# scrubbbbs/cbird

Hardware: AMD Instinct MI355X
Metric: Hamming comparisons/sec + images hashed/sec, 1M-image index, 1/2/4/8 MI355X (higher is better)
Workload: dtype u64 hashes as 64 x FP4 signs, f32 accumulate (find, exact) / u8+f32 (hash)

## Files before the change

cbird_amd/csrc/cbh_internal.h:

```cpp
#pragma once
#include <hip/hip_runtime.h>
#include <stddef.h>
#include <stdint.h>

#include <cstring>
#include <atomic>
#include <map>
#include <memory>
#include <mutex>
#include <utility>
#include <vector>

#include "cbird_hip.h"

namespace cbh {

void combiner_drop(const void* handle);
void set_last_error(const char* where, hipError_t e);
void set_last_error_text(const char* text);
void clear_last_error();
void set_last_error_code(int code);
void* fail_handle(int code, const char* why);

hipError_t malloc_async(void** p, size_t bytes, hipStream_t s);
// ... 80 lines not shown
  JoinCache* join = nullptr;
  std::shared_ptr<const JoinTables>* join_hold = nullptr;
  const JoinNeedles* join_needles = nullptr;
};
int launch_hamm64_scan(const uint64_t* d_hashes, const uint32_t* d_ids, size_t n,
                       const uint64_t* d_q, size_t nq, int thresh, cbh_record* d_rec, size_t cap,
                       unsigned long long* d_total, hipStream_t stream, const ScanOpts& opts = {});
bool scan_takes_mfma(size_t n, size_t nq, int thresh);
int scan_pick_pre(const uint64_t* d_hashes, size_t n, size_t n_total, const uint64_t* d_q, size_t nq, int thresh,
                  hipStream_t stream);
int set_scan_mfma(int mode);
int get_scan_mfma();
void set_scan_pre_max(int t);
void set_scan_pre_rate(int e9);
void set_scan_pre48(int v);
long long get_scan_pre_mask();
long long get_scan_pre48_mask();
long long get_scan_probes();
long long get_scan_probe_rate_e9();
long long get_scan_probe_true_e9();
long long get_scan_probe_rate48_e9();

struct LoneBlock {
  volatile unsigned long long done;
  unsigned long long count;
  static constexpr unsigned kRecs = 512;
  cbh_record recs[kRecs];
};
int launch_find_one(const uint64_t* d_hashes, const uint32_t* d_ids, size_t n, uint64_t q, int thresh, unsigned* d_state,
                    LoneBlock* h_block, unsigned long long seq, hipStream_t stream);
int wait_find_one(const LoneBlock* h_block, unsigned long long seq, hipStream_t stream);

int launch_hamm64_scan_mfma(const uint64_t* d_hashes, const uint32_t* d_ids, size_t n, const uint64_t* d_q, size_t nq,
                            int thresh, cbh_record* d_rec, size_t cap, unsigned long long* d_total, hipStream_t stream,
                            int pre, const ScanOpts& opts);
int expand_needles_for_scan(const uint64_t* d_q, size_t nq, hipStream_t stream, uint4** qx);
constexpr int kProbeMaxThresh = 8;
bool probe_fold_rates(const uint64_t* d_hashes, size_t n, const uint64_t* d_q, size_t nq, int thresh, hipStream_t stream,
                      double* r_cand, double* r_true, double* r_cand48);
int selftest_fp4_products(float* d_out, hipStream_t stream);
constexpr int kJoinMaxThresh = 8;
long long get_scan_joins();
long long get_join_needle_preps();
int set_join_resident(int v);
int set_join_resident_mb(int v);
int get_join_resident();
int get_join_resident_mb();
struct JoinTables {
  int m = 0, device = 0;
  size_t n = 0, bytes = 0;
  uint32_t *hist_h = nullptr, *start_h = nullptr, *hid = nullptr;
  uint64_t* hx = nullptr;
  JoinTables() = default;
  JoinTables(const JoinTables&) = delete;
// ... 148 lines not shown
```

cbird_amd/csrc/cbird_hip.hip:

```cpp
#include <algorithm>
#include <atomic>
#include <cmath>
#include <cstdio>
#include <cstring>
#include <map>
#include <mutex>
#include <new>
#include <string>
#include <vector>

#include "cbh_internal.h"

namespace cbh {

static thread_local std::string t_last_error;
static thread_local int t_last_code = CBH_OK;

void set_last_error(const char* where, hipError_t e) {
  char buf[512];
  snprintf(buf, sizeof buf, "%s: %s (%d)", where, hipGetErrorString(e), (int)e);
  t_last_error = buf;
  t_last_code = e == hipErrorOutOfMemory ? CBH_E_NOMEM : CBH_E_HIP;
}

// ... 1288 lines not shown
      {"fdct_host_vote", [](int v) { g_fdct_host_vote = v; }},
      {"video_host_reduce", [](int v) { g_video_host_reduce = v; }},
      {"orb_retain_order", [](int v) { set_orb_retain_order(v); }},
      {"pool_keep_mb", [](int v) { set_pool_keep_mb(v); }},
      {"pool_live_keep_mb", [](int v) { set_pool_live_keep_mb(v); }},
      {"shard_force_rccl", [](int v) { set_shard_force_rccl(v); }},
      {"shard_exchange", [](int v) { set_shard_exchange(v); }},
      {"fault_alloc_after", [](int v) { set_fault_alloc_after(v); }},
      {"fault_alloc_sticky", [](int v) { set_fault_alloc_sticky(v); }},
      {"fault_driver_oom", [](int v) { set_fault_driver_oom(v); }},
      {"fault_persist_oom", [](int v) { set_fault_persist_oom(v); }},
      {"fault_rccl", [](int v) { set_fault_rccl(v); }},
  };
  if (!strcmp(key, "orb_retain_order") && value != 0 && value != 1) return CBH_E_INVAL;
  if (!strcmp(key, "scan_mfma")) return set_scan_mfma(value);
  if (!strcmp(key, "scan256_mfma")) return set_scan256_mfma(value);
  if (!strcmp(key, "scan256_small")) return set_scan256_small(value);
  if (!strcmp(key, "join_resident")) return set_join_resident(value);
  if (!strcmp(key, "join_resident_mb")) return set_join_resident_mb(value);
  if (!strcmp(key, "color_create_group")) return set_cd_group(value);
  if (!strcmp(key, "scan256_kernels")) {
    if (value != 0) return CBH_E_INVAL;
    clear_scan256_kernels();
    return CBH_OK;
  }
  for (const auto& k : kKnobs)
    if (!strcmp(key, k.name)) {
      k.set(value);
      return CBH_OK;
    }
  return CBH_E_INVAL;
}

int cbh_get_tuning(const char* key, long long* value) {
  if (!key || !value) return CBH_E_INVAL;
  if (!strcmp(key, "fault_alloc_after")) return *value = get_fault_alloc_after(), CBH_OK;
  if (!strcmp(key, "fault_fired")) return *value = (long long)get_fault_fired(), CBH_OK;
  if (!strcmp(key, "alloc_calls")) return *value = (long long)get_alloc_calls(), CBH_OK;
  if (!strncmp(key, "arena_", 6)) return arena_counter(key + 6, value);
  if (!strcmp(key, "scan_mfma")) return *value = get_scan_mfma(), CBH_OK;
  if (!strcmp(key, "scan_pre_mask")) return *value = get_scan_pre_mask(), CBH_OK;
  if (!strcmp(key, "scan_pre48_mask")) return *value = get_scan_pre48_mask(), CBH_OK;
  if (!strcmp(key, "scan256_mfma")) return *value = get_scan256_mfma(), CBH_OK;
  if (!strcmp(key, "scan256_small")) return *value = get_scan256_small(), CBH_OK;
  if (!strcmp(key, "scan256_kernels")) return *value = get_scan256_kernels(), CBH_OK;
  if (!strcmp(key, "color_create_group")) return *value = get_cd_group(), CBH_OK;
  if (!strcmp(key, "color_create_group_last")) return *value = get_cd_group_last(), CBH_OK;
  if (!strcmp(key, "scan_probes")) return *value = get_scan_probes(), CBH_OK;
  if (!strcmp(key, "scan_joins")) return *value = get_scan_joins(), CBH_OK;
  if (!strcmp(key, "join_needle_preps")) return *value = get_join_needle_preps(), CBH_OK;
  if (!strcmp(key, "join_resident")) return *value = get_join_resident(), CBH_OK;
  if (!strcmp(key, "join_resident_mb")) return *value = get_join_resident_mb(), CBH_OK;
  if (!strcmp(key, "slices_on_device")) return *value = get_slices_on_device(), CBH_OK;
  if (!strcmp(key, "scan_probe_rate_e9")) return *value = get_scan_probe_rate_e9(), CBH_OK;
  if (!strcmp(key, "scan_probe_true_e9")) return *value = get_scan_probe_true_e9(), CBH_OK;
  if (!strcmp(key, "scan_probe_rate48_e9")) return *value = get_scan_probe_rate48_e9(), CBH_OK;
  return CBH_E_INVAL;
}


int cbh_idx64_time_scan_dev(cbh_idx64* idx, const void* d_q, size_t nq, int thresh,
                            void* d_records, size_t cap, void* d_total, int iters, float* ms_avg) {
  if (!idx || !ms_avg || iters <= 0 || !d_total) return CBH_E_INVAL;
  if (idx->shards) return CBH_E_UNSUPPORTED;
  DeviceGuard g(idx->device);
  if (!g.ok) return CBH_E_NODEVICE;
  int rc;
  WsLease L(idx, &rc);
  if (!L.ws) return rc;
  hipStream_t s = L.ws->stream;
  hipEvent_t e0, e1;
// ... 99 lines not shown
```

cbird_amd/csrc/fp4_sign.h:

```cpp
#pragma once
#include <hip/hip_runtime.h>

#include <cstdint>

namespace cbh {

typedef int v8i __attribute__((ext_vector_type(8)));
typedef float v16f __attribute__((ext_vector_type(16)));

constexpr int kScaleOne = 0x7f7f7f7f;

__device__ __forceinline__ uint4 fp4_expand32(uint32_t w) {
  uint32_t o[4];
#pragma unroll
  for (int d = 0; d < 4; ++d) {
    uint32_t x = (w >> (8 * d)) & 0xffu;
    x = (x | (x << 12)) & 0x000f000fu;
    x = (x | (x << 6)) & 0x03030303u;
    x = (x | (x << 3)) & 0x11111111u;
    o[d] = 0xaaaaaaaau ^ (x << 3);
  }
  return make_uint4(o[0], o[1], o[2], o[3]);
}

// ... 4 lines not shown
#pragma unroll
  for (int d = 0; d < 2; ++d) {
    uint32_t x = (w >> (8 * d)) & 0xffu;
    x = (x | (x << 12)) & 0x000f000fu;
    x = (x | (x << 6)) & 0x03030303u;
    x = (x | (x << 3)) & 0x11111111u;
    o[d] = (0x88888888u | (mag * 0x11111111u)) ^ (x << 3);
  }
  return make_uint2(o[0], o[1]);
}

__host__ __device__ __forceinline__ uint32_t pre48_sub(uint32_t lo, uint32_t hi, uint32_t k) {
  return k == 0 ? (lo ^ hi) & 0xffffu : k == 1 ? lo >> 16 : hi >> 16;
}

__device__ __forceinline__ v8i fp4_operand(uint4 e) {
  return v8i{(int)e.x, (int)e.y, (int)e.z, (int)e.w, 0, 0, 0, 0};
}

}
```

cbird_amd/csrc/hamm64_mfma.hip:

```cpp
#include <algorithm>
#include <mutex>
#include <vector>

#include "cbh_internal.h"
#include "fp4_sign.h"

namespace cbh {
namespace {

typedef _Float16 h2 __attribute__((ext_vector_type(2)));

constexpr int kThreads = 256;
constexpr int kWaves = 4;
constexpr int kHT = 8;
constexpr int kHT48 = 6;
constexpr int kG = 2;
constexpr float kC0 = 8388608.0f + 16448.0f + 2097152.0f;
constexpr int kScale15 = 0x8e8e8e8e;
constexpr uint32_t kQueue = 2048;
constexpr uint32_t kFlagMaskPre = (1u << 5) | (1u << 11) | (1u << 17) | (1u << 23);
constexpr int kScaleHalf = 0x7e7e7e7e;
constexpr int kScale5 = (int)0x84848484;
constexpr int kScale11 = (int)0x8a8a8a8a;
constexpr int kScale17 = (int)0x90909090;
constexpr int kScale1 = (int)0x80808080;
constexpr int kScale7p = (int)0x86868686;
constexpr int kScale10 = (int)0x89898989;
constexpr int kScale13 = (int)0x8c8c8c8c;
constexpr int kScale19 = (int)0x92929292;

constexpr uint32_t kNeedlePad = 384;
__global__ __launch_bounds__(256) void k_expand_needles(const uint64_t* __restrict__ q, uint32_t nq,
                                                        uint32_t nq_pad, uint4* __restrict__ qx) {
  const uint32_t i = blockIdx.x * 256u + threadIdx.x;
  if (i >= 3u * nq_pad + nq_pad / 128u * 192u) return;
  const uint32_t* w = reinterpret_cast<const uint32_t*>(q);
  if (i < 2u * nq_pad) {
    qx[i] = fp4_expand32((i >> 1) < nq ? w[i] : 0u);
  } else if (i >= 3u * nq_pad) {
    const uint32_t u = i - 3u * nq_pad, quad = u / 192u, m = (u % 192u) >> 6, c = u & 31u, kb = (u >> 5) & 1u;
    uint2 o[2];
#pragma unroll
    for (uint32_t k = 0; k < 2; ++k) {
      const uint32_t s = 2u * (2u * m + kb) + k, j = quad * 128u + (s / 3u) * 32u + c;
      const uint32_t lo = j < nq ? w[2u * j] : 0u, hi = j < nq ? w[2u * j + 1u] : 0u;
      o[k] = fp4_expand16(pre48_sub(lo, hi, s % 3u), s == 3u || s == 7u || s == 9u ? kFp4Four : kFp4Half);
    }
    qx[i] = make_uint4(o[0].x, o[0].y, o[1].x, o[1].y);
  } else {
    const uint32_t j = i - 2u * nq_pad;
    qx[i] = fp4_expand32(j < nq ? w[2u * j] ^ w[2u * j + 1u] : 0u);
  }
// ... 151 lines not shown
  uint32_t* s_out = PRE ? s_queue + kOutOff : s_out2_[PRE ? 0 : wave];
  uint32_t nout = 0;

  v8i a[HT];
#pragma unroll
  for (int t = 0; t < HT; ++t) {
    const uint32_t row = (tile0 + t) * 32u + r;
    const uint2 hv = row < n ? hay[row] : make_uint2(0u, 0u);
    if constexpr (PRE == 2) {
      const uint32_t e0 = pre48_sub(hv.x, hv.y, 0), e1 = pre48_sub(hv.x, hv.y, 1), e2 = pre48_sub(hv.x, hv.y, 2);
      const uint2 s0 = fp4_expand16(half ? e2 : e0, kFp4Half);
      const uint2 s1 = fp4_expand16(half ? e0 : e1, half ? kFp4Four : kFp4Half);
      const uint2 s2 = fp4_expand16(half ? e1 : e2, kFp4Half);
      const uint2 s3 = fp4_expand16(half ? e2 : e0, half ? kFp4Half : kFp4Four);
      a[t] = v8i{(int)s0.x, (int)s0.y, (int)s1.x, (int)s1.y, (int)s2.x, (int)s2.y, (int)s3.x, (int)s3.y};
    } else {
      a[t] = fp4_operand(fp4_expand32(PRE ? hv.x ^ hv.y : (half ? hv.y : hv.x)));
    }
    if (PRE && half == 0) s_hay[t * 32 + r] = hv;
  }
  wave_order();
  v16f c0;
#pragma unroll
  for (int g = 0; g < 16; ++g)
    c0[g] = PRE == 2 ? 8388608.0f + (float)((8u + thresh) * 266305u)
            : PRE  ? 8388608.0f + (float)((16u + (thresh - 1u)) * 266305u) : kC0;
  asm volatile("" : "+v"(c0));
  int scale_b = PRE == 2 ? kScale1 : PRE ? (half ? kScale5 : kScaleHalf) : kScaleOne;
  int scale_b2 = PRE == 2 ? (half ? kScale10 : kScale7p) : PRE ? (half ? kScale17 : kScale11) : kScale15;
  int scale_b3 = half ? kScale19 : kScale13;
  asm volatile("" : "+v"(scale_b));
  asm volatile("" : "+v"(scale_b2));
  if constexpr (PRE == 2) asm volatile("" : "+v"(scale_b3));

  const uint32_t p0 = blockIdx.y * pairs_per_chunk;
  const uint32_t p1 = min(n_pairs, p0 + pairs_per_chunk);
  const uint4* __restrict__ qp = qx + ((size_t)p0 * 64u + r) * 2u + half;
  const uint32_t lo_zero = 0x4080u;
  const uint32_t hi_zero = 0x4B40u;
  const uint32_t lo_thr = lo_zero - 2u * (thresh - 1u);
  const uint32_t hi_thr = hi_zero - (thresh - 1u);
  const uint32_t lo_key = lo_thr << 16, hi_key = hi_thr << 16;
  const HitParams hp = {lo_key, hi_key, lo_zero, hi_zero, thresh, n, nq, keep0, q, ids, rec, cap, total, hay, qmask};

  uint32_t npend = 0;
  uint32_t nitem = 0;
  uint32_t* s_item = s_queue + kItemOff;
// ... 114 lines not shown
        const v8i& h = a[t0 + t];
        c[t] = __builtin_amdgcn_mfma_scale_f32_32x32x64_f8f6f4(v8i{h[2], h[3], h[4], h[5], 0, 0, 0, 0}, b1, c[t], 4, 4, 0,
                                                               kScaleOne, 0, scale_b2);
      }
#pragma unroll
      for (int t = 0; t < G; ++t) {
        const v8i& h = a[t0 + t];
        c[t] = __builtin_amdgcn_mfma_scale_f32_32x32x64_f8f6f4(v8i{h[4], h[5], h[6], h[7], 0, 0, 0, 0}, b2, c[t], 4, 4, 0,
                                                               kScaleOne, 0, scale_b3);
      }
      detect(c, (uint32_t)(t0 / G), p);
    }
    if (npend >= 64u) drain(false);
  };

  auto step = [&](const uint32_t p, const uint4& nA, const uint4& nB) __attribute__((always_inline)) {
    const v8i bA = fp4_operand(nA);
    const v8i bB = fp4_operand(nB);
#pragma unroll
    for (int t0 = 0; t0 < HT; t0 += G) {
      v16f c[G];
#pragma unroll
      for (int t = 0; t < G; ++t)
        c[t] = __builtin_amdgcn_mfma_scale_f32_32x32x64_f8f6f4(a[t0 + t], bA, c0, 4, 4, 0, kScaleOne,
                                                               0, scale_b);
#pragma unroll
      for (int t = 0; t < G; ++t)
        c[t] = __builtin_amdgcn_mfma_scale_f32_32x32x64_f8f6f4(a[t0 + t], bB, c[t], 4, 4, 0,
                                                               kScaleOne, 0, scale_b2);
      if constexpr (PRE != 0) {
// ... 7 lines not shown
            m0 = pkmax3(m0, as_h2(c[t][g]), as_h2(c[t][g + 1]));
            m1 = pkmax3(m1, as_h2(c[t][g + 2]), as_h2(c[t][g + 3]));
          }
        const uint32_t mb = __builtin_bit_cast(uint32_t, __builtin_elementwise_maximum(m0, m1));
        const bool hit = (mb << 16) >= lo_key || mb >= hi_key;
        if (__builtin_amdgcn_ballot_w64(hit) != 0) {
#pragma unroll
          for (int t = 0; t < G; ++t) handle_tile2(c[t], (tile0 + t0 + t) * 32u, p, hp, s_queue, s_out, nout);
        }
      }
    }
    if constexpr (PRE != 0)
      if (npend >= 64u) drain(false);
  };

  (void)step, (void)step48, (void)detect;
  if constexpr (PRE == 2) {
    typedef unsigned v4u_t __attribute__((ext_vector_type(4)));
    const __amdgpu_buffer_rsrc_t rsrc = __builtin_amdgcn_make_buffer_rsrc(
        const_cast<uint4*>(qf + (size_t)(p0 >> 1) * 192u), 0, (int)0xffffffffu, 0x27000);
    const uint32_t voff = lane * 16u;
    auto ldt = [&](uint32_t rel, uint32_t m) -> uint4 {
      const v4u_t v = __builtin_amdgcn_raw_buffer_load_b128(rsrc, (int)voff, (int)(rel * 3072u + m * 1024u), 0);
      return make_uint4(v.x, v.y, v.z, v.w);
    };
    const uint32_t nqd = (p1 - p0 + 1u) >> 1;
    uint4 x0 = ldt(0, 0), x1 = ldt(0, 1), x2 = ldt(0, 2);
#pragma unroll 1
    for (uint32_t rel = 0; rel < nqd; rel += 2) {
      const uint32_t ry = min(rel + 1, nqd - 1);
      const uint4 y0 = ldt(ry, 0), y1 = ldt(ry, 1), y2 = ldt(ry, 2);
      step48(p0 + 2u * rel, x0, x1, x2);
// ... 46 lines not shown
  }
  out_flush(s_out, nout, hp);
}

#define CBH_MFMA_PARAMS                                                                                              \
  const uint2 *__restrict__ hay, const uint32_t *__restrict__ ids, uint32_t n, const uint64_t *__restrict__ q,       \
      const uint4 *__restrict__ qx, uint32_t nq, uint32_t n_pairs, uint32_t pairs_per_chunk, uint32_t thresh,        \
      cbh_record *__restrict__ rec, unsigned long long cap, unsigned long long *__restrict__ total, uint32_t keep0,  \
      const uint2 *__restrict__ qmask, const uint4 *__restrict__ qf
#define CBH_MFMA_ARGS hay, ids, n, q, qx, nq, n_pairs, pairs_per_chunk, thresh, rec, cap, total, keep0, qmask, qf
template <bool PRE>
__global__ __launch_bounds__(kThreads, PRE ? 4 : 1) void k_hamm64_mfma(CBH_MFMA_PARAMS) {
  hamm64_mfma_body<PRE ? 1 : 0>(CBH_MFMA_ARGS);
}
__global__ __launch_bounds__(kThreads, 3) void k_hamm64_mfma48(CBH_MFMA_PARAMS) { hamm64_mfma_body<2>(CBH_MFMA_ARGS); }
#undef CBH_MFMA_PARAMS
#undef CBH_MFMA_ARGS


constexpr uint32_t kFlagMask3 = (1u << 7) | (1u << 14) | (1u << 21);
constexpr int kScale7 = (int)0x86868686;
constexpr int kScale14 = (int)0x8d8d8d8d;

__device__ __forceinline__ void handle_tile3(const v16f& c, uint32_t row0, uint32_t p3, const HitParams& hp,
                                             uint32_t* s_queue, uint32_t* s_out, uint32_t& nout) {
  const uint32_t lane = threadIdx.x & 63u;
  uint32_t any = 0;
#pragma unroll
  for (int g = 0; g < 16; ++g) any |= as_u32(c[g]);
  if (__builtin_amdgcn_ballot_w64((any & kFlagMask3) != 0) == 0) return;
// ... 115 lines not shown
  }
  out_flush(s_out, nout, hp);
}

constexpr uint32_t kProbeS = 2048;
constexpr int kProbeT = kProbeMaxThresh;

__device__ __forceinline__ uint32_t probe_mix(uint32_t x) {
  x = ((x >> 16) ^ x) * 0x45d9f3bu;
  x = ((x >> 16) ^ x) * 0x45d9f3bu;
  return (x >> 16) ^ x;
}
__global__ __launch_bounds__(256) void k_fold_probe(const uint2* __restrict__ hay, uint32_t n, const uint2* __restrict__ q,
                                                    uint32_t nq, uint32_t sh, uint32_t sq, uint32_t* __restrict__ counts) {
  __shared__ uint2 s_h[64];
  __shared__ uint32_t s_cnt[3 * kProbeT];
  const uint32_t t = threadIdx.x;
  if (t < 64) {
    const uint32_t i = blockIdx.y * 64u + t;
    s_h[t] = i < sh ? hay[sh == n ? i : probe_mix(i) % n] : make_uint2(0u, 0u);
  }
  if (t < 3 * kProbeT) s_cnt[t] = 0;
  __syncthreads();
  const uint32_t j = blockIdx.x * 256u + t;
  const uint32_t nslots = min(64u, sh - blockIdx.y * 64u);
  uint32_t cnt[kProbeT] = {}, cnt64[kProbeT] = {}, cnt48[kProbeT] = {};
  if (j < sq) {
    const uint2 nv = q[sq == nq ? j : probe_mix(j ^ 0x9e3779b9u) % nq];
    const uint32_t f = nv.x ^ nv.y;
    for (uint32_t k = 0; k < nslots; ++k) {
      const uint2 hv = s_h[k];
      const uint32_t d = (uint32_t)__popc(f ^ hv.x ^ hv.y);
#pragma unroll
      for (int th = 0; th < kProbeT; ++th) cnt[th] += d < (uint32_t)(th + 1) ? 1u : 0u;
      const uint32_t d48 = (uint32_t)__popc((f ^ hv.x ^ hv.y) & 0xffffu) + (uint32_t)__popc((nv.x ^ hv.x) >> 16) +
                           (uint32_t)__popc((nv.y ^ hv.y) >> 16);
#pragma unroll
      for (int th = 0; th < kProbeT; ++th) cnt48[th] += d48 <= (uint32_t)(th + 1) || d48 > (uint32_t)(th + 33) ? 1u : 0u;
      if (d < (uint32_t)kProbeT) {
        const uint32_t d64 = (uint32_t)__popc(nv.x ^ hv.x) + (uint32_t)__popc(nv.y ^ hv.y);
#pragma unroll
        for (int th = 0; th < kProbeT; ++th) cnt64[th] += d64 < (uint32_t)(th + 1) ? 1u : 0u;
      }
    }
  }
#pragma unroll
  for (int th = 0; th < 3 * kProbeT; ++th) {
    uint32_t v = th < kProbeT ? cnt[th % kProbeT] : th < 2 * kProbeT ? cnt64[th % kProbeT] : cnt48[th % kProbeT];
#pragma unroll
    for (int o = 32; o > 0; o >>= 1) v += __shfl_down(v, o);
    if ((t & 63u) == 0 && v) atomicAdd(&s_cnt[th], v);
  }
  __syncthreads();
  if (t < 3 * kProbeT && s_cnt[t]) atomicAdd(&counts[t], s_cnt[t]);
}

__device__ __forceinline__ uint32_t selftest_fp4_code(uint32_t i) {
  return ((i >> 1) == 0 ? kFp4Half : (i >> 1) == 1 ? 0x2u : kFp4Four) | ((i & 1u) << 3);
}
__global__ __launch_bounds__(64) void k_selftest_fp4(float* __restrict__ out) {
  const uint32_t lane = threadIdx.x, half = lane >> 5;
  for (uint32_t i = 0; i < 720u; ++i) {
    const uint32_t kb = i & 1u, ci = (i >> 1) & 1u, k = (i >> 2) % 5u, ib = (i / 20u) % 6u, ia = i / 120u;
    const uint32_t fa = selftest_fp4_code(ia) * (ci ? 0x11111111u : 1u), fb = selftest_fp4_code(ib) * (ci ? 0x11111111u : 1u);
    const bool on = half == kb;
    const v8i a = {on ? (int)fa : 0, on && ci ? (int)fa : 0, 0, 0, 0, 0, 0, 0};
    const v8i b = {on ? (int)fb : 0, on && ci ? (int)fb : 0, 0, 0, 0, 0, 0, 0};
    int sc = k == 0 ? kScale1 : k == 1 ? kScale7p : k == 2 ? kScale10 : k == 3 ? kScale13 : kScale19;
    asm volatile("" : "+v"(sc));
// ... 4 lines not shown
  }
}

std::mutex g_probe_mu;
std::vector<uint32_t*> g_probe_free;
uint32_t* probe_slot_get() {
  {
    std::lock_guard<std::mutex> lk(g_probe_mu);
    if (!g_probe_free.empty()) {
      uint32_t* p = g_probe_free.back();
      g_probe_free.pop_back();
      return p;
    }
  }
  uint32_t* p = nullptr;
  if (hipHostMalloc(&p, 3 * kProbeT * sizeof(uint32_t)) != hipSuccess) {
    (void)hipGetLastError();
    return nullptr;
  }
  return p;
}
void probe_slot_put(uint32_t* p) {
  std::lock_guard<std::mutex> lk(g_probe_mu);
  g_probe_free.push_back(p);
}

}

bool probe_fold_rates(const uint64_t* d_hashes, size_t n, const uint64_t* d_q, size_t nq, int thresh, hipStream_t stream,
                      double* r_cand, double* r_true, double* r_cand48) {
  uint32_t* d_cnt = nullptr;
  if (cbh::malloc_async((void**)&d_cnt, 3 * kProbeT * sizeof(uint32_t), stream) != hipSuccess) {
    (void)hipGetLastError();
    return false;
  }
  uint32_t* h_cnt = probe_slot_get();
  bool ok = h_cnt != nullptr;
  const uint32_t sh = (uint32_t)std::min<size_t>(n, kProbeS), sq = (uint32_t)std::min<size_t>(nq, kProbeS);
  if (ok) {
    ok = hipMemsetAsync(d_cnt, 0, 3 * kProbeT * sizeof(uint32_t), stream) == hipSuccess;
    if (ok) {
      hipLaunchKernelGGL(k_fold_probe, dim3((sq + 255u) / 256u, (sh + 63u) / 64u), dim3(256), 0, stream,
                         reinterpret_cast<const uint2*>(d_hashes), (uint32_t)n, reinterpret_cast<const uint2*>(d_q),
                         (uint32_t)nq, sh, sq, d_cnt);
      ok = hipGetLastError() == hipSuccess &&
           hipMemcpyAsync(h_cnt, d_cnt, 3 * kProbeT * sizeof(uint32_t), hipMemcpyDeviceToHost, stream) == hipSuccess &&
           hipStreamSynchronize(stream) == hipSuccess;
    }
  }
  (void)cbh::free_async(d_cnt, stream);
  if (ok) {
    const double pairs = (double)sh * (double)sq;
    *r_cand = (double)h_cnt[thresh - 1] / pairs;
    *r_true = (double)h_cnt[kProbeT + thresh - 1] / pairs;
    *r_cand48 = (double)h_cnt[2 * kProbeT + thresh - 1] / pairs;
  } else {
    (void)hipGetLastError();
  }
  if (h_cnt) probe_slot_put(h_cnt);
  return ok;
}

int selftest_fp4_products(float* d_out, hipStream_t stream) {
  hipLaunchKernelGGL(k_selftest_fp4, dim3(1), dim3(64), 0, stream, d_out);
  CBH_HIP(hipGetLastError());
  return CBH_OK;
}

static uint32_t padded_needles(size_t nq) { return (uint32_t)((nq + kNeedlePad - 1) / kNeedlePad) * kNeedlePad; }

int expand_needles_for_scan(const uint64_t* d_q, size_t nq, hipStream_t stream, uint4** qx_out) {
  *qx_out = nullptr;
  if (nq == 0 || nq > CBH_MAX_QUERIES_PER_CALL) return CBH_OK;
  const uint32_t nq_pad = padded_needles(nq);
  uint4* qx = nullptr;
  CBH_HIP(malloc_async((void**)&qx, (size_t)nq_pad * 72u, stream));
  hipLaunchKernelGGL(k_expand_needles, dim3((3u * nq_pad + nq_pad / 128u * 192u + 255u) / 256u), dim3(256), 0, stream, d_q,
                     (uint32_t)nq, nq_pad, qx);
  hipError_t e = hipGetLastError();
  if (e != hipSuccess) {
    (void)free_async(qx, stream);
    CBH_HIP(e);
  }
  *qx_out = qx;
  return CBH_OK;
}

int launch_hamm64_scan_mfma(const uint64_t* d_hashes, const uint32_t* d_ids, size_t n, const uint64_t* d_q, size_t nq,
                            int thresh, cbh_record* d_rec, size_t cap, unsigned long long* d_total, hipStream_t stream,
                            int pre, const ScanOpts& o) {
  const uint32_t n_pairs = (uint32_t)((nq + 63) / 64);
  const uint32_t n_triples = (uint32_t)((nq + 95) / 96);
  const uint32_t nq_pad = padded_needles(nq);
  const uint4* qx = o.qx;
  uint4* qx_own = nullptr;
  if (!qx) {
    int rc = expand_needles_for_scan(d_q, nq, stream, &qx_own);
    if (rc) return rc;
    qx = qx_own;
  }
  const uint4* qf = qx + (pre == 2 ? 3u : 2u) * (size_t)nq_pad;
  const uint32_t rows_per_wg = 32u * (pre == 2 ? kHT48 : kHT) * kWaves;
  const uint32_t sib = std::max(1u, o.siblings);
  const uint32_t wgs = (uint32_t)((n + rows_per_wg - 1) / rows_per_wg);
  if (!pre && thresh <= 64) {
    uint32_t tpc = 172u;
    while (tpc > 11 && (uint64_t)wgs * sib * ((n_triples + tpc - 1) / tpc) < 8192) tpc = (tpc + 1) / 2;
    uint32_t ch3 = (n_triples + tpc - 1) / tpc;
    if (ch3 > 65535) {
      tpc = (n_triples + 65534) / 65535;
      ch3 = (n_triples + tpc - 1) / tpc;
    }
    hipLaunchKernelGGL(k_hamm64_mfma3, dim3(wgs, ch3), dim3(kThreads), 0, stream,
                       reinterpret_cast<const uint2*>(d_hashes), d_ids, (uint32_t)n, d_q, qx, (uint32_t)nq, n_triples, tpc,
                       (uint32_t)thresh, d_rec, (unsigned long long)cap, d_total, (uint32_t)o.keep_id0,
                       reinterpret_cast<const uint2*>(o.d_qmask));
  } else {
    uint32_t ppc = pre ? 512u : 256u;
    while (ppc > 16 && (uint64_t)wgs * sib * ((n_pairs + ppc - 1) / ppc) < 8192) ppc >>= 1;
    uint32_t chunks = (n_pairs + ppc - 1) / ppc;
    if (chunks > 65535) {
      ppc = ((n_pairs + 65534) / 65535 + 1u) & ~1u;
      chunks = (n_pairs + ppc - 1) / ppc;
    }
#define CBH_MFMA(K)                                                                                                   \
  hipLaunchKernelGGL(K, dim3(wgs, chunks), dim3(kThreads), 0, stream,                                                 \
                     reinterpret_cast<const uint2*>(d_hashes), d_ids, (uint32_t)n, d_q, qx, (uint32_t)nq, n_pairs, ppc, \
                     (uint32_t)thresh, d_rec, (unsigned long long)cap, d_total, (uint32_t)o.keep_id0,                 \
                     reinterpret_cast<const uint2*>(o.d_qmask), qf)
    if (pre == 2) CBH_MFMA(k_hamm64_mfma48); else if (pre) CBH_MFMA((k_hamm64_mfma<true>)); else CBH_MFMA((k_hamm64_mfma<false>));
#undef CBH_MFMA
  }
  hipError_t e = hipGetLastError();
  if (qx_own) (void)cbh::free_async(qx_own, stream);
  CBH_HIP(e);
  return CBH_OK;
}

}
```

cbird_amd/csrc/hamm64_scan.hip:

```cpp
#include <atomic>

#include "cbh_internal.h"

namespace cbh {
namespace {

constexpr int kThreads = 256;
constexpr int kH = 8;
constexpr int kQB = 8;

__device__ __forceinline__ uint32_t min3u(uint32_t a, uint32_t b, uint32_t c) {
  return min(min(a, b), c);
}

__device__ __forceinline__ void emit(cbh_record* __restrict__ rec, unsigned long long cap,
                                     unsigned long long* __restrict__ total, uint32_t qidx,
                                     uint32_t dist, uint32_t id) {
  unsigned long long slot = atomicAdd(total, 1ull);
  if (slot < cap) rec[slot] = ((cbh_record)qidx << 39) | ((cbh_record)dist << 32) | id;
}

template <int H>
__device__ __forceinline__ void exact_block(const uint2 (&h)[H], uint32_t base_idx, uint32_t n,
                                            const uint32_t* __restrict__ ids,
// ... 253 lines not shown
#if defined(__x86_64__)
    __builtin_ia32_pause();
#endif
  }
}

namespace {

constexpr int kPreMax = 7;
constexpr size_t kMfmaMinNq = 256;
constexpr size_t kMfmaMinN = 4096;
constexpr int kPreStatic = 6;
constexpr double kTrueWeight = 8.0;
constexpr double kSlopePre = 1.3e4, kBaseFull = 15.75, kTrueFull = 2.7e5, kTruePre = 0.7e5;
constexpr double kBasePre = 8.55, kBase48 = 14.0, kSlope48 = 2.8e4, kTrue48 = 1.0e5, kPre48Margin = 0.9;
constexpr int kPre48MaxThresh = 16;
constexpr uint64_t kProbeMinPairs = 1ull << 31;

int g_scan_mfma = 1;
int g_pre_max_thresh = -1;
int g_pre_rate_max_e9 = 300000;
int g_pre48 = -1;
std::atomic<uint64_t> g_pre_mask{0};
std::atomic<uint64_t> g_pre48_mask{0};
std::atomic<uint64_t> g_n_probe{0};
std::atomic<long long> g_last_rate_e9{-1};
std::atomic<long long> g_last_true_e9{-1};
std::atomic<long long> g_last_rate48_e9{-1};

enum class Join { None, IfCheaper, Forced };
enum class Kernel { PopcEq, PopcPre, PopcFull, Mfma };
struct Route {
  Join join;
  Kernel kernel;
  double scan_ms;
};

Route route(size_t n, size_t nq, int thresh, bool masked) {
  Route r;
  r.scan_ms = (double)n * (double)nq * (thresh <= 5 ? 8.7e-12 : thresh == 6 ? 9.7e-12 : thresh == 7 ? 12.1e-12 : 15.8e-12);
  const bool joinable = thresh <= kJoinMaxThresh && !masked && n < 0xfffffff0ull;
  r.join = !joinable ? Join::None : g_scan_mfma == 4 ? Join::Forced
           : g_scan_mfma == 3 && r.scan_ms >= 1.0 ? Join::IfCheaper : Join::None;
  const bool mfma = thresh <= 65 && (g_scan_mfma == 2 || g_scan_mfma == 4 ||
                                     (g_scan_mfma != 0 && nq >= kMfmaMinNq && n >= kMfmaMinN));
  r.kernel = mfma ? Kernel::Mfma : thresh == 1 ? Kernel::PopcEq : thresh <= kPreMax ? Kernel::PopcPre : Kernel::PopcFull;
  return r;
}

int launch_popc(Kernel kernel, const uint64_t* d_hashes, const uint32_t* d_ids, size_t n, const uint64_t* d_q, size_t nq,
                int thresh, cbh_record* d_rec, size_t cap, unsigned long long* d_total, hipStream_t stream,
                const ScanOpts& o) {
  const uint32_t tile = kThreads * kH;
  const uint32_t tiles = (uint32_t)((n + tile - 1) / tile);
  uint32_t q_chunk = 16384;
  while (q_chunk > 1024 && (uint64_t)tiles * ((nq + q_chunk - 1) / q_chunk) < 8192) q_chunk >>= 1;
  uint32_t chunks = (uint32_t)((nq + q_chunk - 1) / q_chunk);
  if (chunks > 65535) {
// ... 15 lines not shown
  return CBH_OK;
}

}

bool scan_takes_mfma(size_t n, size_t nq, int thresh) {
  return thresh >= 1 && route(n, nq, thresh, false).kernel == Kernel::Mfma;
}

bool scan_routes_to_join(size_t n, size_t nq, int thresh, bool masked) {
  return thresh >= 1 && n >= 1 && nq >= 1 && route(n, nq, thresh, masked).join != Join::None;
}

int scan_pick_pre(const uint64_t* d_hashes, size_t n, size_t n_total, const uint64_t* d_q, size_t nq, int thresh,
                  hipStream_t stream) {
  if (g_pre48 == 1 && thresh <= kPre48MaxThresh) return 2;
  if (thresh > 32) return 0;
  if (g_pre_max_thresh >= 0) return thresh <= g_pre_max_thresh;
  if (thresh > kProbeMaxThresh) return 0;
  if ((uint64_t)n_total * (uint64_t)nq < kProbeMinPairs) return thresh <= kPreStatic;
  double r_cand = 0, r_true = 0, r48 = 0;
  if (!probe_fold_rates(d_hashes, n, d_q, nq, thresh, stream, &r_cand, &r_true, &r48)) return thresh <= kPreStatic;
  g_last_rate_e9 = (long long)(r_cand * 1e9);
  g_last_true_e9 = (long long)(r_true * 1e9);
  g_last_rate48_e9 = (long long)(r48 * 1e9);
  g_n_probe++;
  const double d_pre = kSlopePre * (r_cand - kTrueWeight * r_true - (double)g_pre_rate_max_e9 * 1e-9);
  const bool pre = d_pre <= 0;
  if (g_pre48 != 0) {
    const double t_48 = kBase48 + kSlope48 * r48 + kTrue48 * r_true;
    const double t_pre = kBasePre + kSlopePre * r_cand + kTruePre * r_true, t_full = kBaseFull + kTrueFull * r_true;
    if (pre ? t_48 < kPre48Margin * t_pre : t_48 < t_full) return 2;
  }
  return pre;
}

namespace {

int launch_zero_needles(const uint64_t* d_hashes, const uint32_t* d_ids, size_t n, const uint64_t* d_q, size_t nq,
                        int thresh, cbh_record* d_rec, size_t cap, unsigned long long* d_total, hipStream_t stream,
                        const ScanOpts& o) {
  Scratch scratch(stream);
  uint32_t* list = nullptr;
  CBH_HIP(scratch.get(&list, (nq + 1) * sizeof(uint32_t)));
  CBH_HIP(hipMemsetAsync(list, 0, sizeof(uint32_t), stream));
  hipLaunchKernelGGL(k_zero_needle_list, dim3((unsigned)((nq + 255) / 256)), dim3(256), 0, stream, d_q, (uint32_t)nq, list);
// ... 23 lines not shown
namespace {

int scan_nonzero_needles(const uint64_t* d_hashes, const uint32_t* d_ids, size_t n, const uint64_t* d_q, size_t nq,
                         int thresh, cbh_record* d_rec, size_t cap, unsigned long long* d_total, hipStream_t stream,
                         const ScanOpts& o) {
  const Route r = route(n, nq, thresh, o.d_qmask != nullptr);
  if (r.join != Join::None) {
    const bool force = r.join == Join::Forced;
    const int rc = launch_hamm64_join(d_hashes, d_ids, n, d_q, nq, thresh, d_rec, cap, d_total, stream, o, force, r.scan_ms);
    if (rc == CBH_OK || force || (rc != CBH_E_UNSUPPORTED && rc != CBH_E_NOMEM)) return rc;
    if (rc == CBH_E_NOMEM) cbh_clear_error();
  }
  if (r.kernel != Kernel::Mfma) return launch_popc(r.kernel, d_hashes, d_ids, n, d_q, nq, thresh, d_rec, cap, d_total, stream, o);
  const int pre = o.pre >= 0 ? o.pre : scan_pick_pre(d_hashes, n, n, d_q, nq, thresh, stream);
  if (thresh < 64) {
    if (pre == 1) g_pre_mask |= 1ull << thresh; else g_pre_mask &= ~(1ull << thresh);
    if (pre == 2) g_pre48_mask |= 1ull << thresh; else g_pre48_mask &= ~(1ull << thresh);
  }
  return launch_hamm64_scan_mfma(d_hashes, d_ids, n, d_q, nq, thresh, d_rec, cap, d_total, stream, pre, o);
}

}

int set_scan_mfma(int mode) {
  if (mode < 0 || mode > 4) return CBH_E_INVAL;
  g_scan_mfma = mode;
  return CBH_OK;
}
int get_scan_mfma() { return g_scan_mfma; }
void set_scan_pre_max(int t) {
  if (t >= -1 && t <= 32) g_pre_max_thresh = t;
}
void set_scan_pre_rate(int e9) {
  if (e9 >= 0) g_pre_rate_max_e9 = e9;
}
void set_scan_pre48(int v) {
  if (v >= -1 && v <= 1) g_pre48 = v;
}
long long get_scan_pre_mask() { return (long long)g_pre_mask.load(); }
long long get_scan_pre48_mask() { return (long long)g_pre48_mask.load(); }
long long get_scan_probes() { return (long long)g_n_probe.load(); }
long long get_scan_probe_rate_e9() { return g_last_rate_e9.load(); }
long long get_scan_probe_true_e9() { return g_last_true_e9.load(); }
long long get_scan_probe_rate48_e9() { return g_last_rate48_e9.load(); }

}
```

Before: 86280 billion.

## Add 16-bit folded prefilter MFMA scan path chosen by probe cost model

Adds a third prefilter mode that folds each 64-bit hash into 16 bits (XOR of all four 16-bit quarters) and runs a single FP4 MFMA per needle to reject candidates before the exact check. The idea is that a Hamming distance within the threshold survives the fold, so the cheaper 16-bit screen removes most of the matrix work of the existing 32-bit fold path. The fold-rate probe now also measures the 16-bit candidate rate, and a cost model picks the new kernel when its estimated time beats the 32-bit prefilter. Route's scan-cost estimate for thresh 1 is also lowered, which changes join-versus-scan decisions. In exchange, the weaker fold lets through more false candidates that must be verified, and needle expansion needs a larger buffer.

After: 88690 billion, median of 6. 1.03x the previous value.

```diff
diff --git a/cbird_amd/csrc/cbh_internal.h b/cbird_amd/csrc/cbh_internal.h
--- a/cbird_amd/csrc/cbh_internal.h
+++ b/cbird_amd/csrc/cbh_internal.h
@@ -118,12 +118,15 @@
 void set_scan_pre_max(int t);
 void set_scan_pre_rate(int e9);
 void set_scan_pre48(int v);
+int set_scan_pre16(int v);
 long long get_scan_pre_mask();
 long long get_scan_pre48_mask();
+long long get_scan_pre16_mask();
 long long get_scan_probes();
 long long get_scan_probe_rate_e9();
 long long get_scan_probe_true_e9();
 long long get_scan_probe_rate48_e9();
+long long get_scan_probe_rate16_e9();
 
 struct LoneBlock {
   volatile unsigned long long done;
@@ -135,13 +138,14 @@
                     LoneBlock* h_block, unsigned long long seq, hipStream_t stream);
 int wait_find_one(const LoneBlock* h_block, unsigned long long seq, hipStream_t stream);
 
+constexpr int kPre16MaxThresh = 8;
 int launch_hamm64_scan_mfma(const uint64_t* d_hashes, const uint32_t* d_ids, size_t n, const uint64_t* d_q, size_t nq,
                             int thresh, cbh_record* d_rec, size_t cap, unsigned long long* d_total, hipStream_t stream,
                             int pre, const ScanOpts& opts);
 int expand_needles_for_scan(const uint64_t* d_q, size_t nq, hipStream_t stream, uint4** qx);
 constexpr int kProbeMaxThresh = 8;
 bool probe_fold_rates(const uint64_t* d_hashes, size_t n, const uint64_t* d_q, size_t nq, int thresh, hipStream_t stream,
-                      double* r_cand, double* r_true, double* r_cand48);
+                      double* r_cand, double* r_true, double* r_cand48, double* r_cand16);
 int selftest_fp4_products(float* d_out, hipStream_t stream);
 constexpr int kJoinMaxThresh = 8;
 long long get_scan_joins();
diff --git a/cbird_amd/csrc/cbird_hip.hip b/cbird_amd/csrc/cbird_hip.hip
--- a/cbird_amd/csrc/cbird_hip.hip
+++ b/cbird_amd/csrc/cbird_hip.hip
@@ -1326,6 +1326,7 @@
   };
   if (!strcmp(key, "orb_retain_order") && value != 0 && value != 1) return CBH_E_INVAL;
   if (!strcmp(key, "scan_mfma")) return set_scan_mfma(value);
+  if (!strcmp(key, "scan_pre16")) return set_scan_pre16(value);
   if (!strcmp(key, "scan256_mfma")) return set_scan256_mfma(value);
   if (!strcmp(key, "scan256_small")) return set_scan256_small(value);
   if (!strcmp(key, "join_resident")) return set_join_resident(value);
@@ -1353,6 +1354,7 @@
   if (!strcmp(key, "scan_mfma")) return *value = get_scan_mfma(), CBH_OK;
   if (!strcmp(key, "scan_pre_mask")) return *value = get_scan_pre_mask(), CBH_OK;
   if (!strcmp(key, "scan_pre48_mask")) return *value = get_scan_pre48_mask(), CBH_OK;
+  if (!strcmp(key, "scan_pre16_mask")) return *value = get_scan_pre16_mask(), CBH_OK;
   if (!strcmp(key, "scan256_mfma")) return *value = get_scan256_mfma(), CBH_OK;
   if (!strcmp(key, "scan256_small")) return *value = get_scan256_small(), CBH_OK;
   if (!strcmp(key, "scan256_kernels")) return *value = get_scan256_kernels(), CBH_OK;
@@ -1367,6 +1369,7 @@
   if (!strcmp(key, "scan_probe_rate_e9")) return *value = get_scan_probe_rate_e9(), CBH_OK;
   if (!strcmp(key, "scan_probe_true_e9")) return *value = get_scan_probe_true_e9(), CBH_OK;
   if (!strcmp(key, "scan_probe_rate48_e9")) return *value = get_scan_probe_rate48_e9(), CBH_OK;
+  if (!strcmp(key, "scan_probe_rate16_e9")) return *value = get_scan_probe_rate16_e9(), CBH_OK;
   return CBH_E_INVAL;
 }
 
diff --git a/cbird_amd/csrc/fp4_sign.h b/cbird_amd/csrc/fp4_sign.h
--- a/cbird_amd/csrc/fp4_sign.h
+++ b/cbird_amd/csrc/fp4_sign.h
@@ -42,6 +42,11 @@
   return k == 0 ? (lo ^ hi) & 0xffffu : k == 1 ? lo >> 16 : hi >> 16;
 }
 
+__host__ __device__ __forceinline__ uint32_t fold16(uint32_t lo, uint32_t hi) {
+  const uint32_t f = lo ^ hi;
+  return (f ^ (f >> 16)) & 0xffffu;
+}
+
 __device__ __forceinline__ v8i fp4_operand(uint4 e) {
   return v8i{(int)e.x, (int)e.y, (int)e.z, (int)e.w, 0, 0, 0, 0};
 }
diff --git a/cbird_amd/csrc/hamm64_mfma.hip b/cbird_amd/csrc/hamm64_mfma.hip
--- a/cbird_amd/csrc/hamm64_mfma.hip
+++ b/cbird_amd/csrc/hamm64_mfma.hip
@@ -33,9 +33,16 @@
 __global__ __launch_bounds__(256) void k_expand_needles(const uint64_t* __restrict__ q, uint32_t nq,
                                                         uint32_t nq_pad, uint4* __restrict__ qx) {
   const uint32_t i = blockIdx.x * 256u + threadIdx.x;
-  if (i >= 3u * nq_pad + nq_pad / 128u * 192u) return;
+  const uint32_t o16 = 3u * nq_pad + nq_pad / 128u * 192u;
+  if (i >= o16 + nq_pad / 128u * 64u) return;
   const uint32_t* w = reinterpret_cast<const uint32_t*>(q);
-  if (i < 2u * nq_pad) {
+  if (i >= o16) {
+    const uint32_t u = i - o16, c = u & 31u, kb = (u >> 5) & 1u;
+    const uint32_t j0 = (u >> 6) * 128u + kb * 64u + c, j1 = j0 + 32u;
+    const uint2 lo = fp4_expand16(j0 < nq ? fold16(w[2u * j0], w[2u * j0 + 1u]) : 0u, kFp4Half);
+    const uint2 hi = fp4_expand16(j1 < nq ? fold16(w[2u * j1], w[2u * j1 + 1u]) : 0u, kFp4Four);
+    qx[i] = make_uint4(lo.x, lo.y, hi.x, hi.y);
+  } else if (i < 2u * nq_pad) {
     qx[i] = fp4_expand32((i >> 1) < nq ? w[i] : 0u);
   } else if (i >= 3u * nq_pad) {
     const uint32_t u = i - 3u * nq_pad, quad = u / 192u, m = (u % 192u) >> 6, c = u & 31u, kb = (u >> 5) & 1u;
@@ -217,6 +224,10 @@
       const uint2 s2 = fp4_expand16(half ? e1 : e2, kFp4Half);
       const uint2 s3 = fp4_expand16(half ? e2 : e0, half ? kFp4Half : kFp4Four);
       a[t] = v8i{(int)s0.x, (int)s0.y, (int)s1.x, (int)s1.y, (int)s2.x, (int)s2.y, (int)s3.x, (int)s3.y};
+    } else if constexpr (PRE == 3) {
+      const uint32_t f = fold16(hv.x, hv.y);
+      const uint2 s0 = fp4_expand16(f, kFp4Half), s1 = fp4_expand16(f, kFp4Four);
+      a[t] = v8i{(int)s0.x, (int)s0.y, (int)s1.x, (int)s1.y, 0, 0, 0, 0};
     } else {
       a[t] = fp4_operand(fp4_expand32(PRE ? hv.x ^ hv.y : (half ? hv.y : hv.x)));
     }
@@ -226,14 +237,15 @@
   v16f c0;
 #pragma unroll
   for (int g = 0; g < 16; ++g)
-    c0[g] = PRE == 2 ? 8388608.0f + (float)((8u + thresh) * 266305u)
+    c0[g] = PRE == 3 ? 8388608.0f + (float)((24u + (thresh - 1u)) * 266305u)
+            : PRE == 2 ? 8388608.0f + (float)((8u + thresh) * 266305u)
             : PRE  ? 8388608.0f + (float)((16u + (thresh - 1u)) * 266305u) : kC0;
   asm volatile("" : "+v"(c0));
-  int scale_b = PRE == 2 ? kScale1 : PRE ? (half ? kScale5 : kScaleHalf) : kScaleOne;
+  int scale_b = PRE == 3 ? (half ? kScale13 : kScale1) : PRE == 2 ? kScale1 : PRE ? (half ? kScale5 : kScaleHalf) : kScaleOne;
   int scale_b2 = PRE == 2 ? (half ? kScale10 : kScale7p) : PRE ? (half ? kScale17 : kScale11) : kScale15;
   int scale_b3 = half ? kScale19 : kScale13;
   asm volatile("" : "+v"(scale_b));
-  asm volatile("" : "+v"(scale_b2));
+  if constexpr (PRE != 3) asm volatile("" : "+v"(scale_b2));
   if constexpr (PRE == 2) asm volatile("" : "+v"(scale_b3));
 
   const uint32_t p0 = blockIdx.y * pairs_per_chunk;
@@ -378,6 +390,19 @@
     if (npend >= 64u) drain(false);
   };
 
+  auto step16 = [&](const uint32_t p, const uint4& nn) __attribute__((always_inline)) {
+    const v8i bq = fp4_operand(nn);
+#pragma unroll
+    for (int t0 = 0; t0 < HT; t0 += G) {
+      v16f c[G];
+#pragma unroll
+      for (int t = 0; t < G; ++t)
+        c[t] = __builtin_amdgcn_mfma_scale_f32_32x32x64_f8f6f4(a[t0 + t], bq, c0, 4, 4, 0, kScaleOne, 0, scale_b);
+      detect(c, (uint32_t)(t0 / G), p);
+    }
+    if (npend >= 64u) drain(false);
+  };
+
   auto step = [&](const uint32_t p, const uint4& nA, const uint4& nB) __attribute__((always_inline)) {
     const v8i bA = fp4_operand(nA);
     const v8i bB = fp4_operand(nB);
@@ -415,8 +440,29 @@
       if (npend >= 64u) drain(false);
   };
 
-  (void)step, (void)step48, (void)detect;
-  if constexpr (PRE == 2) {
+  (void)step, (void)step48, (void)step16, (void)detect, (void)scale_b2, (void)scale_b3;
+  if constexpr (PRE == 3) {
+    typedef unsigned v4u_t __attribute__((ext_vector_type(4)));
+    const __amdgpu_buffer_rsrc_t rsrc = __builtin_amdgcn_make_buffer_rsrc(
+        const_cast<uint4*>(qf + (size_t)(p0 >> 1) * 64u), 0, (int)0xffffffffu, 0x27000);
+    const uint32_t voff = lane * 16u;
+    auto ldt = [&](uint32_t rel) -> uint4 {
+      const v4u_t v = __builtin_amdgcn_raw_buffer_load_b128(rsrc, (int)voff, (int)(rel * 1024u), 0);
+      return make_uint4(v.x, v.y, v.z, v.w);
+    };
+    const uint32_t nqd = (p1 - p0 + 1u) >> 1;
+    uint4 x0 = ldt(0);
+#pragma unroll 1
+    for (uint32_t rel = 0; rel < nqd; rel += 2) {
+      const uint4 y0 = ldt(min(rel + 1, nqd - 1));
+      step16(p0 + 2u * rel, x0);
+      if (rel + 1 < nqd) {
+        x0 = ldt(min(rel + 2, nqd - 1));
+        step16(p0 + 2u * rel + 2u, y0);
+      }
+    }
+    if (npend | nitem) drain(true);
+  } else if constexpr (PRE == 2) {
     typedef unsigned v4u_t __attribute__((ext_vector_type(4)));
     const __amdgpu_buffer_rsrc_t rsrc = __builtin_amdgcn_make_buffer_rsrc(
         const_cast<uint4*>(qf + (size_t)(p0 >> 1) * 192u), 0, (int)0xffffffffu, 0x27000);
@@ -493,6 +539,7 @@
   hamm64_mfma_body<PRE ? 1 : 0>(CBH_MFMA_ARGS);
 }
 __global__ __launch_bounds__(kThreads, 3) void k_hamm64_mfma48(CBH_MFMA_PARAMS) { hamm64_mfma_body<2>(CBH_MFMA_ARGS); }
+__global__ __launch_bounds__(kThreads, 4) void k_hamm64_mfma16(CBH_MFMA_PARAMS) { hamm64_mfma_body<3>(CBH_MFMA_ARGS); }
 #undef CBH_MFMA_PARAMS
 #undef CBH_MFMA_ARGS
 
@@ -638,17 +685,17 @@
 __global__ __launch_bounds__(256) void k_fold_probe(const uint2* __restrict__ hay, uint32_t n, const uint2* __restrict__ q,
                                                     uint32_t nq, uint32_t sh, uint32_t sq, uint32_t* __restrict__ counts) {
   __shared__ uint2 s_h[64];
-  __shared__ uint32_t s_cnt[3 * kProbeT];
+  __shared__ uint32_t s_cnt[4 * kProbeT];
   const uint32_t t = threadIdx.x;
   if (t < 64) {
     const uint32_t i = blockIdx.y * 64u + t;
     s_h[t] = i < sh ? hay[sh == n ? i : probe_mix(i) % n] : make_uint2(0u, 0u);
   }
-  if (t < 3 * kProbeT) s_cnt[t] = 0;
+  if (t < 4 * kProbeT) s_cnt[t] = 0;
   __syncthreads();
   const uint32_t j = blockIdx.x * 256u + t;
   const uint32_t nslots = min(64u, sh - blockIdx.y * 64u);
-  uint32_t cnt[kProbeT] = {}, cnt64[kProbeT] = {}, cnt48[kProbeT] = {};
+  uint32_t cnt[kProbeT] = {}, cnt64[kProbeT] = {}, cnt48[kProbeT] = {}, cnt16[kProbeT] = {};
   if (j < sq) {
     const uint2 nv = q[sq == nq ? j : probe_mix(j ^ 0x9e3779b9u) % nq];
     const uint32_t f = nv.x ^ nv.y;
@@ -661,6 +708,9 @@
                            (uint32_t)__popc((nv.y ^ hv.y) >> 16);
 #pragma unroll
       for (int th = 0; th < kProbeT; ++th) cnt48[th] += d48 <= (uint32_t)(th + 1) || d48 > (uint32_t)(th + 33) ? 1u : 0u;
+      const uint32_t x32 = f ^ hv.x ^ hv.y, d16 = (uint32_t)__popc((x32 ^ (x32 >> 16)) & 0xffffu);
+#pragma unroll
+      for (int th = 0; th < kProbeT; ++th) cnt16[th] += d16 < (uint32_t)(th + 1) ? 1u : 0u;
       if (d < (uint32_t)kProbeT) {
         const uint32_t d64 = (uint32_t)__popc(nv.x ^ hv.x) + (uint32_t)__popc(nv.y ^ hv.y);
 #pragma unroll
@@ -669,14 +719,15 @@
     }
   }
 #pragma unroll
-  for (int th = 0; th < 3 * kProbeT; ++th) {
-    uint32_t v = th < kProbeT ? cnt[th % kProbeT] : th < 2 * kProbeT ? cnt64[th % kProbeT] : cnt48[th % kProbeT];
+  for (int th = 0; th < 4 * kProbeT; ++th) {
+    uint32_t v = th < kProbeT ? cnt[th % kProbeT] : th < 2 * kProbeT ? cnt64[th % kProbeT]
+                 : th < 3 * kProbeT ? cnt48[th % kProbeT] : cnt16[th % kProbeT];
 #pragma unroll
     for (int o = 32; o > 0; o >>= 1) v += __shfl_down(v, o);
     if ((t & 63u) == 0 && v) atomicAdd(&s_cnt[th], v);
   }
   __syncthreads();
-  if (t < 3 * kProbeT && s_cnt[t]) atomicAdd(&counts[t], s_cnt[t]);
+  if (t < 4 * kProbeT && s_cnt[t]) atomicAdd(&counts[t], s_cnt[t]);
 }
 
 __device__ __forceinline__ uint32_t selftest_fp4_code(uint32_t i) {
@@ -711,7 +762,7 @@
     }
   }
   uint32_t* p = nullptr;
-  if (hipHostMalloc(&p, 3 * kProbeT * sizeof(uint32_t)) != hipSuccess) {
+  if (hipHostMalloc(&p, 4 * kProbeT * sizeof(uint32_t)) != hipSuccess) {
     (void)hipGetLastError();
     return nullptr;
   }
@@ -725,9 +776,9 @@
 }
 
 bool probe_fold_rates(const uint64_t* d_hashes, size_t n, const uint64_t* d_q, size_t nq, int thresh, hipStream_t stream,
-                      double* r_cand, double* r_true, double* r_cand48) {
+                      double* r_cand, double* r_true, double* r_cand48, double* r_cand16) {
   uint32_t* d_cnt = nullptr;
-  if (cbh::malloc_async((void**)&d_cnt, 3 * kProbeT * sizeof(uint32_t), stream) != hipSuccess) {
+  if (cbh::malloc_async((void**)&d_cnt, 4 * kProbeT * sizeof(uint32_t), stream) != hipSuccess) {
     (void)hipGetLastError();
     return false;
   }
@@ -735,13 +786,13 @@
   bool ok = h_cnt != nullptr;
   const uint32_t sh = (uint32_t)std::min<size_t>(n, kProbeS), sq = (uint32_t)std::min<size_t>(nq, kProbeS);
   if (ok) {
-    ok = hipMemsetAsync(d_cnt, 0, 3 * kProbeT * sizeof(uint32_t), stream) == hipSuccess;
+    ok = hipMemsetAsync(d_cnt, 0, 4 * kProbeT * sizeof(uint32_t), stream) == hipSuccess;
     if (ok) {
       hipLaunchKernelGGL(k_fold_probe, dim3((sq + 255u) / 256u, (sh + 63u) / 64u), dim3(256), 0, stream,
                          reinterpret_cast<const uint2*>(d_hashes), (uint32_t)n, reinterpret_cast<const uint2*>(d_q),
                          (uint32_t)nq, sh, sq, d_cnt);
       ok = hipGetLastError() == hipSuccess &&
-           hipMemcpyAsync(h_cnt, d_cnt, 3 * kProbeT * sizeof(uint32_t), hipMemcpyDeviceToHost, stream) == hipSuccess &&
+           hipMemcpyAsync(h_cnt, d_cnt, 4 * kProbeT * sizeof(uint32_t), hipMemcpyDeviceToHost, stream) == hipSuccess &&
            hipStreamSynchronize(stream) == hipSuccess;
     }
   }
@@ -751,6 +802,7 @@
     *r_cand = (double)h_cnt[thresh - 1] / pairs;
     *r_true = (double)h_cnt[kProbeT + thresh - 1] / pairs;
     *r_cand48 = (double)h_cnt[2 * kProbeT + thresh - 1] / pairs;
+    *r_cand16 = (double)h_cnt[3 * kProbeT + thresh - 1] / pairs;
   } else {
     (void)hipGetLastError();
   }
@@ -771,8 +823,8 @@
   if (nq == 0 || nq > CBH_MAX_QUERIES_PER_CALL) return CBH_OK;
   const uint32_t nq_pad = padded_needles(nq);
   uint4* qx = nullptr;
-  CBH_HIP(malloc_async((void**)&qx, (size_t)nq_pad * 72u, stream));
-  hipLaunchKernelGGL(k_expand_needles, dim3((3u * nq_pad + nq_pad / 128u * 192u + 255u) / 256u), dim3(256), 0, stream, d_q,
+  CBH_HIP(malloc_async((void**)&qx, (size_t)nq_pad * 80u, stream));
+  hipLaunchKernelGGL(k_expand_needles, dim3((5u * nq_pad + 255u) / 256u), dim3(256), 0, stream, d_q,
                      (uint32_t)nq, nq_pad, qx);
   hipError_t e = hipGetLastError();
   if (e != hipSuccess) {
@@ -786,6 +838,7 @@
 int launch_hamm64_scan_mfma(const uint64_t* d_hashes, const uint32_t* d_ids, size_t n, const uint64_t* d_q, size_t nq,
                             int thresh, cbh_record* d_rec, size_t cap, unsigned long long* d_total, hipStream_t stream,
                             int pre, const ScanOpts& o) {
+  if (pre == 3 && thresh > kPre16MaxThresh) return CBH_E_INVAL;
   const uint32_t n_pairs = (uint32_t)((nq + 63) / 64);
   const uint32_t n_triples = (uint32_t)((nq + 95) / 96);
   const uint32_t nq_pad = padded_needles(nq);
@@ -796,7 +849,7 @@
     if (rc) return rc;
     qx = qx_own;
   }
-  const uint4* qf = qx + (pre == 2 ? 3u : 2u) * (size_t)nq_pad;
+  const uint4* qf = qx + (pre == 3 ? 3u * (size_t)nq_pad + nq_pad / 128u * 192u : (pre == 2 ? 3u : 2u) * (size_t)nq_pad);
   const uint32_t rows_per_wg = 32u * (pre == 2 ? kHT48 : kHT) * kWaves;
   const uint32_t sib = std::max(1u, o.siblings);
   const uint32_t wgs = (uint32_t)((n + rows_per_wg - 1) / rows_per_wg);
@@ -825,7 +878,7 @@
                      reinterpret_cast<const uint2*>(d_hashes), d_ids, (uint32_t)n, d_q, qx, (uint32_t)nq, n_pairs, ppc, \
                      (uint32_t)thresh, d_rec, (unsigned long long)cap, d_total, (uint32_t)o.keep_id0,                 \
                      reinterpret_cast<const uint2*>(o.d_qmask), qf)
-    if (pre == 2) CBH_MFMA(k_hamm64_mfma48); else if (pre) CBH_MFMA((k_hamm64_mfma<true>)); else CBH_MFMA((k_hamm64_mfma<false>));
+    if (pre == 3) CBH_MFMA(k_hamm64_mfma16); else if (pre == 2) CBH_MFMA(k_hamm64_mfma48); else if (pre) CBH_MFMA((k_hamm64_mfma<true>)); else CBH_MFMA((k_hamm64_mfma<false>));
 #undef CBH_MFMA
   }
   hipError_t e = hipGetLastError();
diff --git a/cbird_amd/csrc/hamm64_scan.hip b/cbird_amd/csrc/hamm64_scan.hip
--- a/cbird_amd/csrc/hamm64_scan.hip
+++ b/cbird_amd/csrc/hamm64_scan.hip
@@ -291,6 +291,7 @@
 constexpr double kTrueWeight = 8.0;
 constexpr double kSlopePre = 1.3e4, kBaseFull = 15.75, kTrueFull = 2.7e5, kTruePre = 0.7e5;
 constexpr double kBasePre = 8.55, kBase48 = 14.0, kSlope48 = 2.8e4, kTrue48 = 1.0e5, kPre48Margin = 0.9;
+constexpr double kBase16 = 5.85, kPre16Margin = 0.9;
 constexpr int kPre48MaxThresh = 16;
 constexpr uint64_t kProbeMinPairs = 1ull << 31;
 
@@ -298,12 +299,15 @@
 int g_pre_max_thresh = -1;
 int g_pre_rate_max_e9 = 300000;
 int g_pre48 = -1;
+int g_pre16 = -1;
 std::atomic<uint64_t> g_pre_mask{0};
 std::atomic<uint64_t> g_pre48_mask{0};
+std::atomic<uint64_t> g_pre16_mask{0};
 std::atomic<uint64_t> g_n_probe{0};
 std::atomic<long long> g_last_rate_e9{-1};
 std::atomic<long long> g_last_true_e9{-1};
 std::atomic<long long> g_last_rate48_e9{-1};
+std::atomic<long long> g_last_rate16_e9{-1};
 
 enum class Join { None, IfCheaper, Forced };
 enum class Kernel { PopcEq, PopcPre, PopcFull, Mfma };
@@ -315,10 +319,12 @@
 
 Route route(size_t n, size_t nq, int thresh, bool masked) {
   Route r;
-  r.scan_ms = (double)n * (double)nq * (thresh <= 5 ? 8.7e-12 : thresh == 6 ? 9.7e-12 : thresh == 7 ? 12.1e-12 : 15.8e-12);
+  const double pairs = (double)n * (double)nq;
+  const double pre_ms = pairs * (thresh <= 5 ? 8.7e-12 : thresh == 6 ? 9.7e-12 : thresh == 7 ? 12.1e-12 : 15.8e-12);
+  r.scan_ms = thresh == 1 ? pairs * 6.1e-12 : pre_ms;
   const bool joinable = thresh <= kJoinMaxThresh && !masked && n < 0xfffffff0ull;
   r.join = !joinable ? Join::None : g_scan_mfma == 4 ? Join::Forced
-           : g_scan_mfma == 3 && r.scan_ms >= 1.0 ? Join::IfCheaper : Join::None;
+           : g_scan_mfma == 3 && pre_ms >= 1.0 ? Join::IfCheaper : Join::None;
   const bool mfma = thresh <= 65 && (g_scan_mfma == 2 || g_scan_mfma == 4 ||
                                      (g_scan_mfma != 0 && nq >= kMfmaMinNq && n >= kMfmaMinN));
   r.kernel = mfma ? Kernel::Mfma : thresh == 1 ? Kernel::PopcEq : thresh <= kPreMax ? Kernel::PopcPre : Kernel::PopcFull;
@@ -364,22 +370,27 @@
 
 int scan_pick_pre(const uint64_t* d_hashes, size_t n, size_t n_total, const uint64_t* d_q, size_t nq, int thresh,
                   hipStream_t stream) {
+  if (g_pre16 == 1 && thresh <= kPre16MaxThresh) return 3;
   if (g_pre48 == 1 && thresh <= kPre48MaxThresh) return 2;
   if (thresh > 32) return 0;
   if (g_pre_max_thresh >= 0) return thresh <= g_pre_max_thresh;
   if (thresh > kProbeMaxThresh) return 0;
   if ((uint64_t)n_total * (uint64_t)nq < kProbeMinPairs) return thresh <= kPreStatic;
-  double r_cand = 0, r_true = 0, r48 = 0;
-  if (!probe_fold_rates(d_hashes, n, d_q, nq, thresh, stream, &r_cand, &r_true, &r48)) return thresh <= kPreStatic;
+  double r_cand = 0, r_true = 0, r48 = 0, r16 = 0;
+  if (!probe_fold_rates(d_hashes, n, d_q, nq, thresh, stream, &r_cand, &r_true, &r48, &r16)) return thresh <= kPreStatic;
   g_last_rate_e9 = (long long)(r_cand * 1e9);
   g_last_true_e9 = (long long)(r_true * 1e9);
   g_last_rate48_e9 = (long long)(r48 * 1e9);
+  g_last_rate16_e9 = (long long)(r16 * 1e9);
   g_n_probe++;
   const double d_pre = kSlopePre * (r_cand - kTrueWeight * r_true - (double)g_pre_rate_max_e9 * 1e-9);
   const bool pre = d_pre <= 0;
+  const double t_pre = kBasePre + kSlopePre * r_cand + kTruePre * r_true, t_full = kBaseFull + kTrueFull * r_true;
+  if (g_pre16 != 0 && pre && thresh <= kPre16MaxThresh &&
+      kBase16 + kSlopePre * r16 + kTruePre * r_true < kPre16Margin * t_pre)
+    return 3;
   if (g_pre48 != 0) {
     const double t_48 = kBase48 + kSlope48 * r48 + kTrue48 * r_true;
-    const double t_pre = kBasePre + kSlopePre * r_cand + kTruePre * r_true, t_full = kBaseFull + kTrueFull * r_true;
     if (pre ? t_48 < kPre48Margin * t_pre : t_48 < t_full) return 2;
   }
   return pre;
@@ -433,8 +444,9 @@
   if (r.kernel != Kernel::Mfma) return launch_popc(r.kernel, d_hashes, d_ids, n, d_q, nq, thresh, d_rec, cap, d_total, stream, o);
   const int pre = o.pre >= 0 ? o.pre : scan_pick_pre(d_hashes, n, n, d_q, nq, thresh, stream);
   if (thresh < 64) {
-    if (pre == 1) g_pre_mask |= 1ull << thresh; else g_pre_mask &= ~(1ull << thresh);
+    if (pre == 1 || pre == 3) g_pre_mask |= 1ull << thresh; else g_pre_mask &= ~(1ull << thresh);
     if (pre == 2) g_pre48_mask |= 1ull << thresh; else g_pre48_mask &= ~(1ull << thresh);
+    if (pre == 3) g_pre16_mask |= 1ull << thresh; else g_pre16_mask &= ~(1ull << thresh);
   }
   return launch_hamm64_scan_mfma(d_hashes, d_ids, n, d_q, nq, thresh, d_rec, cap, d_total, stream, pre, o);
 }
@@ -457,10 +469,17 @@
   if (v >= -1 && v <= 1) g_pre48 = v;
 }
 long long get_scan_pre_mask() { return (long long)g_pre_mask.load(); }
+int set_scan_pre16(int v) {
+  if (v < -1 || v > 1) return CBH_E_INVAL;
+  g_pre16 = v;
+  return CBH_OK;
+}
 long long get_scan_pre48_mask() { return (long long)g_pre48_mask.load(); }
+long long get_scan_pre16_mask() { return (long long)g_pre16_mask.load(); }
 long long get_scan_probes() { return (long long)g_n_probe.load(); }
 long long get_scan_probe_rate_e9() { return g_last_rate_e9.load(); }
 long long get_scan_probe_true_e9() { return g_last_true_e9.load(); }
 long long get_scan_probe_rate48_e9() { return g_last_rate48_e9.load(); }
-
-}
+long long get_scan_probe_rate16_e9() { return g_last_rate16_e9.load(); }
+
+}
```
